# meyer-lab/cmtf-pls

Hardware: AMD Instinct MI355X
Metric: nipals_iters_per_sec (higher is better)
Workload: dtype f32

## Files before the change

cmtf_pls_amd/_lib.py:

```python
from __future__ import annotations

import ctypes
import os
from ctypes import c_char_p, c_double, c_int, c_int64, c_size_t, c_uint32, c_uint64, c_void_p

_HERE = os.path.dirname(os.path.abspath(__file__))
LIB_PATH = os.environ.get("CMTFPLS_LIB") or os.path.join(_HERE, "lib", "libcmtfpls.so")

_P = c_void_p

class XcovBlock(ctypes.Structure):
    _fields_ = [("S", _P), ("S2", _P), ("colcnt", _P), ("n_samples", c_double), ("order", c_int), ("A", c_int), ("B", c_int),
                ("n_squarings", c_int), ("Z", _P), ("wA", _P), ("wB", _P), ("info", _P)]


class KfoldState(ctypes.Structure):
    _fields_ = [("I", c_int), ("A", c_int), ("B", c_int), ("M", c_int), ("K", c_int), ("R", c_int)] + [
        (name, _P) for name in ("fold_of", "S", "mean", "Yk", "Gy", "WA", "WB", "Q", "Wa", "Wb", "T", "Gt", "coef", "Rm", "tm",
                                "Tout", "vec", "n_iter", "status", "part")]


class CvCoupledBlock(ctypes.Structure):
    _fields_ = [("X", _P), ("order", c_int), ("A", c_int), ("B", c_int)]


class LooCoupledBlock(ctypes.Structure):
    _fields_ = [("X", _P), ("colsum", _P), ("order", c_int), ("A", c_int), ("B", c_int)]


SIGNATURES = {
    "cmtfpls_xcov_iterate_blocks_f64": (c_int, [ctypes.POINTER(XcovBlock), c_int, c_int, _P, _P, _P, _P, _P, c_int, _P, c_size_t, _P]),
    "cmtfpls_abi_version": (c_int, []),
    "cmtfpls_last_error": (c_char_p, []),
    "cmtfpls_clear_error": (c_int, []),
    "cmtfpls_status_to_host": (c_int, [_P, _P, c_size_t, _P, _P]),
    "cmtfpls_colstats_workspace_bytes": (c_size_t, [c_int64, c_int64]),
    "cmtfpls_colstats_f32": (c_int, [_P, c_int64, c_int64, _P, _P, _P, c_size_t, _P]),
    "cmtfpls_colstats_f64": (c_int, [_P, c_int64, c_int64, _P, _P, _P, c_size_t, _P]),
    "cmtfpls_sweep_partials": (c_int, []),
    "cmtfpls_center_f32": (c_int, [_P, c_int64, c_int64, _P, _P, _P, _P]),
    "cmtfpls_center_f64": (c_int, [_P, c_int64, c_int64, _P, _P, _P, _P]),
    "cmtfpls_mode0_contract_workspace_bytes": (c_size_t, [c_int64, c_int64]),
# ... 144 lines not shown
                                                                       c_int, c_int]),
    "cmtfpls_loo_xcov_coupled_tensor_lds_bytes": (c_size_t, [ctypes.POINTER(LooCoupledBlock), c_int, ctypes.POINTER(c_int), c_int, c_int,
                                                            c_int]),
    "cmtfpls_loo_xcov_coupled_tensor_f64": (c_int, [ctypes.POINTER(LooCoupledBlock), c_int, ctypes.POINTER(c_int), _P, _P, c_int, c_int, c_int,
                                                    c_double, c_int, c_int, c_int, _P, _P, _P, c_size_t, _P]),
    "cmtfpls_cv_masked_fold_workspace_bytes": (c_size_t, [c_int, c_int, c_int, c_int, c_int]),
    "cmtfpls_cv_masked_f64": (c_int, [_P, _P, _P, c_int, _P, _P, _P, c_int, c_int, c_int, c_int, c_int, c_double, c_int, c_int,
                                      c_int, _P, _P, _P, _P, _P, c_size_t, _P]),
    "cmtfpls_cv_masked_model_workspace_bytes": (c_size_t, [c_int, c_int, c_int, c_int, c_int]),
    "cmtfpls_cv_masked_models_f64": (c_int, [_P, _P, _P, _P, c_int, c_int, c_int, c_int, c_int, c_int, c_double, c_int, c_int, c_int]
                                     + [_P] * 8 + [_P, c_size_t, _P]),
    "cmtfpls_cv_masked_tensor_fold_workspace_bytes": (c_size_t, [c_int] * 6),
    "cmtfpls_cv_masked_tensor_f64": (c_int, [_P, _P, _P, c_int, _P, _P, _P, c_int, c_int, c_int, c_int, c_int, c_int, c_double, c_int,
                                             c_int, c_int, _P, _P, _P, _P, _P, c_size_t, _P]),
    "cmtfpls_cv_masked_tensor_model_workspace_bytes": (c_size_t, [c_int] * 6),
    "cmtfpls_cv_masked_tensor_models_f64": (c_int, [_P, _P, _P, _P, c_int, c_int, c_int, c_int, c_int, c_int, c_int, c_double, c_int,
                                                    c_int, c_int] + [_P] * 9 + [_P, c_size_t, _P]),
    "cmtfpls_cv_masked_coupled_workspace_bytes": (c_size_t, [ctypes.POINTER(CvCoupledBlock), c_int, c_int, c_int, c_int]),
    "cmtfpls_cv_masked_coupled_lds_bytes": (c_size_t, [ctypes.POINTER(CvCoupledBlock), c_int, c_int, c_int, c_int]),
    "cmtfpls_cv_masked_coupled_f64": (c_int, [ctypes.POINTER(CvCoupledBlock), c_int, _P, _P, _P, c_int, c_int, c_int, c_int, c_double,
                                              c_int, c_int, c_int] + [_P] * 8 + [_P, c_size_t, _P]),
    "cmtfpls_fit_small_workspace_bytes": (c_size_t, [c_int, c_int, c_int, c_int]),
    "cmtfpls_fit_small_f64": (c_int, [_P, _P, c_int, c_int, c_int, c_int, c_int, c_double, c_int] + [_P] * 11 + [_P, c_size_t, _P]),
    "cmtfpls_add_noise_f32": (c_int, [_P, c_int64, c_double, c_uint64, c_uint64, c_double, _P]),
    "cmtfpls_add_noise_f64": (c_int, [_P, c_int64, c_double, c_uint64, c_uint64, c_double, _P]),
    "cmtfpls_ceiling_max_blocks": (c_int, []),
    "cmtfpls_ceiling_read": (c_int, [_P, c_size_t, c_int64, c_int, _P, c_int, _P]),
    "cmtfpls_ceiling_rmw": (c_int, [_P, c_size_t, c_int64, c_int, c_int, _P]),
    "cmtfpls_ceiling_copy": (c_int, [_P, _P, c_size_t, c_int64, c_int, c_int, _P]),
}

_lib = None


class CmtfplsError(RuntimeError):
    pass


def load():
    global _lib
    if _lib is not None:
        return _lib
    if not os.path.exists(LIB_PATH):
        raise CmtfplsError(
            f"{LIB_PATH} not found: build the HIP extension first (python -c 'import __graft_entry__ as g; g.build()'). "
            "cmtf_pls_amd has no CPU fallback."
# ... 15 lines not shown
```

cmtf_pls_amd/backend.py:

```python
from __future__ import annotations

import ctypes
from typing import Optional, Tuple

import torch

from . import _lib

_SUFFIX = {torch.float32: "f32", torch.float64: "f64"}


def _ptr(t: Optional[torch.Tensor]):
    return None if t is None else t.data_ptr()


def _int_pairs(pairs):
    flat = [int(v) for p in pairs for v in p]
    return (ctypes.c_int * len(flat))(*flat)


def _scratch(nbytes: int, device) -> torch.Tensor:
    return torch.empty(max(int(nbytes), 256), dtype=torch.uint8, device=device)


# ... 318 lines not shown
        return self._form(rc, "mttkrp", out)

    def score(self, X2, A, B, wA, wB, rowcnt, out) -> torch.Tensor:
        _lib.check(self._fn("score", X2)(_ptr(X2), X2.shape[0], A, B, _ptr(wA), _ptr(wB), _ptr(rowcnt), _ptr(out), self._stream()), "score")
        return out

    def score_s(self, S, A, B, wA, wB, out) -> torch.Tensor:
        assert S.dtype == torch.float64 and S.is_contiguous()
        _lib.check(self.lib.cmtfpls_score_s_f64(_ptr(S), S.shape[0], A, B, _ptr(wA), _ptr(wB), _ptr(out), self._stream()), "score_s")
        return out

    def score_contract(self, X2, A, B, wA, wB, shift, t, Z, sub_own=None, add_other=None, alpha: float = 1.0,
                       csum: Optional[torch.Tensor] = None) -> Optional[torch.Tensor]:
        I, P = X2.shape
        if not X2.is_contiguous() or P != A * B:
            return None
        for v in (sub_own, add_other):
            assert v is None or (v.is_contiguous() and v.numel() == I and v.dtype == torch.float64)
        nbytes = self.lib.cmtfpls_score_contract_workspace_bytes(I, P)
        ws = self._workspace("score_contract", max(nbytes, 256))
        rc = self._fn("score_contract", X2)(_ptr(X2), I, A, B, _ptr(wA), _ptr(wB), _ptr(shift), _ptr(sub_own), _ptr(add_other), float(alpha),
                                            _ptr(t), _ptr(Z), _ptr(csum), _ptr(ws), ws.numel(), self._stream())
        return self._form(rc, "score_contract", Z)

    def score_gram(self, X2, A, B, wA, wB, rowcnt, out, Y: torch.Tensor, qpart: torch.Tensor) -> Optional[torch.Tensor]:
        assert qpart.numel() >= self.n_partials * Y.shape[1] and qpart.is_contiguous()
        rc = self._fn("score_gram", X2)(_ptr(X2), X2.shape[0], A, B, _ptr(wA), _ptr(wB), _ptr(rowcnt), _ptr(out),
                                        _ptr(Y), Y.stride(0), Y.shape[1], _ptr(qpart), self._stream())
        return self._form(rc, "score_gram", out)

    def q_update(self, q: torch.Tensor, qpart: Optional[torch.Tensor] = None, normalize: bool = True,
                 G: Optional[torch.Tensor] = None, q_prev: Optional[torch.Tensor] = None,
                 du2: Optional[torch.Tensor] = None, nparts: Optional[int] = None) -> None:
        M = q.numel()
        nrows = (nparts or self.n_partials) if qpart is not None else 0
        assert qpart is None or (qpart.is_contiguous() and qpart.numel() >= nrows * M)
        _lib.check(self.lib.cmtfpls_q_update_f64(_ptr(qpart), nrows, M, _ptr(q), int(normalize),
                                                 _ptr(G), _ptr(q_prev), _ptr(du2), self._stream()), "q_update")

    def deflate(self, X2, A, B, t, wA, wB) -> torch.Tensor:
        part = self.empty(self.n_partials)
        _lib.check(self._fn("deflate", X2)(_ptr(X2), X2.shape[0], A, B, _ptr(t), _ptr(wA), _ptr(wB), _ptr(part), self._stream()), "deflate")
        return self._close_partials(part)

    def deflate_contract_yq(self, X2, A, B, t, wA, wB, Y: torch.Tensor, q: torch.Tensor, masked: bool,
                            out: torch.Tensor) -> Optional[torch.Tensor]:
# ... 543 lines not shown
```

cmtf_pls_amd/fitrun.py:

```python
from __future__ import annotations

import math
from typing import Dict, List, Optional

import numpy as np
import torch

from .fitrun_xcov import XcovMixin
from .state import BlockState, FitState, split_trailing, validate_limits


class FitRun(XcovMixin):

    def __init__(self, eng: NipalsEngine, Xs: List[torch.Tensor], Y: torch.Tensor, n_components: int, coupled: bool,
                 algorithm: str = "direct", owned: Optional[List[bool]] = None, allow_raw: bool = True):
        be, comm = eng.be, eng.comm
        Xs = list(Xs)
        owned = [True] * len(Xs) if owned is None else list(owned)
        if algorithm not in ("direct", "xcov"):
            raise ValueError("algorithm must be 'direct' or 'xcov'")
        self.algorithm_requested = self.algorithm = algorithm
        self.notes: List[str] = []
        validate_limits([tuple(X.shape) for X in Xs], n_components)
        self.eng, self.Xs, self.Y, self.R, self.coupled = eng, Xs, Y, n_components, coupled
# ... 105 lines not shown
            self.S, self.S2, self.S12 = [], [], []
            for blk in self.blocks:
                if blk.has_miss and self._s_pair:
                    both = be.empty(2 * M, blk.A * blk.B)
                    self.S12.append(both)
                    self.S.append(both[:M])
                    self.S2.append(both[M:])
                else:
                    self.S12.append(None)
                    pre = self._s_prebuilt.get(len(self.S))
                    self.S.append(pre if pre is not None else be.empty(M, blk.A * blk.B))
                    self.S2.append(be.empty(M, blk.A * blk.B) if blk.has_miss else None)
            self.rowscale = [(float(blk.A * blk.B) / blk.rowcnt) if blk.has_miss else None for blk in self.blocks]
            any_miss = any(blk.has_miss for blk in self.blocks)
            self.Yw = be.empty(I, 2 * M if self._s_pair else M) if any_miss else None
            self.Gy = be.empty(M, M)
            self.Tq = be.empty(nb, M)
            self.qx = [be.zeros(M), be.zeros(M)]
            self.qc = self.qx[0]
            self.qn = self.Tq[0] if (nb == 1 and not coupled) else be.empty(M)
            self._s_carry = (not any(blk.has_miss for blk in self.blocks)
                             and all(hasattr(be, f) for f in ("s_downdate", "deflate_contract_yq")))
            self._s_ready = False
            self._nowrite = False
            if self.raw:
                self.zM = be.zeros(M)
                self.zA = [be.zeros(blk.A) for blk in self.blocks]
                self.zB = [be.zeros(blk.B) for blk in self.blocks]
            if self._s_carry:
                self.yhat = be.empty(I, 1)
                self.one = be.empty(1)
                self.one.fill_(1.0)
                self.vs = [be.empty(blk.A * blk.B) for blk in self.blocks]
                self._nowrite = eng.opt.xcov_nowrite and hasattr(be, "kr_axpy") and R <= 64
                if self._nowrite:
                    self.dot_log = be.zeros(R, 1 + len(self.blocks))
                    self.Gw = be.empty(R * R)
                    self._G_last = None
                    self._one_read = R > 1 and eng.opt.xcov_one_read and hasattr(be, "score_contract")
                    if self._one_read:
                        self._fused_b = max(range(len(self.blocks)), key=lambda b: self.blocks[b].A * self.blocks[b].B)
                        P0 = self.blocks[self._fused_b].A * self.blocks[self._fused_b].B
                        self.ps = be.empty(P0)
                        self.Rm = be.zeros(P0, R)
                        self.corr = be.empty(I)
                        self.csum = be.empty(1)
            assert self._nowrite or not self.raw, "an uncentred X needs the form of the loop that never writes it"

    def _blocks_from_one_read(self, Xs: List[torch.Tensor]) -> Optional[List[BlockState]]:
        be, comm = self.eng.be, self.eng.comm
        blocks, n = [], float(self.n_total)
        for b, X in enumerate(Xs):
            I = X.shape[0]
            X2 = X.view(I, -1)
            P = X2.shape[1]
            out = be.xcov_stats(X2, self.Y, out=be.empty(self.M, P))
            if out is None:
                return None
            S, stats = out
            comm.allreduce(stats)
            colsum, colsq = stats[:P], stats[P:]
            ssq = (colsq - colsum * colsum / n).sum().reshape(1)
            if not bool(torch.isfinite(ssq).all().item()):
                return None
            A, B = split_trailing(X.shape)
            blocks.append(BlockState(shape=tuple(X.shape), A=A, B=B, mean=colsum / n, has_miss=False, colcnt=None, rowcnt=None,
                                     ssq0=float("nan"), dtype=X.dtype))
            self._s_prebuilt[b] = S
            self._ssq0_dev[b] = ssq
        return blocks
# ... 17 lines not shown
            if self.S12[b] is not None:
                self.Yw[:, :self.M].copy_(self.Y)
                torch.mul(self.Y, self.rowscale[b][:, None], out=self.Yw[:, self.M:])
                be.xcov(self.X2[b], self.Yw, True, out=self.S12[b], mixed=self.mixed)
                comm.allreduce(self.S12[b])
                continue
            if b in self._s_prebuilt:
                del self._s_prebuilt[b]
            elif self.raw and self._ssq_with_s and b not in self._ssq0_dev:
                _, ssq = be.xcov_ssq(self.X2[b], self.Y, blk.mean, out=self.S[b])
                self._ssq0_dev[b] = comm.allreduce(ssq)
            else:
                be.xcov(self.X2[b], self.Y, blk.has_miss, out=self.S[b], mixed=self.mixed)
            comm.allreduce(self.S[b])
            if self.raw:
                ysum, _ = be.colstats(self.Y)
                comm.allreduce(ysum)
                be.s_downdate(self.S[b], blk.A, blk.B, self.zM, self.zA[b], self.zB[b], ysum, blk.mean)
            if blk.has_miss:
                torch.mul(self.Y, self.rowscale[b][:, None], out=self.Yw)
                be.xcov(self.X2[b], self.Yw, True, out=self.S2[b], mixed=self.mixed)
                comm.allreduce(self.S2[b])
        self._s_ready = False
        be.gram_tn(self.Y, self.Y, out=self.Gy)
        comm.allreduce(self.Gy)
        self._parity = 0
        self.qc = self.qx[0]
        self.qc.zero_()
        self.qc[0] = 1.0

    def inner_loop(self, a: int, max_iter: int, tol: float, verbose: int = 0) -> None:
        if max_iter > 0 and self._pipeline_ok():
            self._pipelined = True
            self._inner_loop_xcov_pipelined(a, max_iter, tol, verbose)
            return
        for it in range(max_iter):
            du = self.iterate(it)
            if du is not None and du < tol:
                if verbose:
                    print("Comp {}: converged after {} iterations".format(a, it))
                break

    def _update_budgets(self, host) -> bool:
        retry = False
        for b in range(len(self.blocks)):
            conv, used = host[1 + 2 * b] > 0.5, int(host[2 + 2 * b])
            if used < 0:
                self._chain_gave_up()
                retry = True
                continue
# ... 349 lines not shown
    def _store_loadings(self, a: int) -> None:
        for b, blk in enumerate(self.blocks):
            if len(blk.shape) == 2:
                blk.loadings[0][:, a].copy_(self.wB[b])
            elif len(blk.shape) == 3:
                blk.loadings[0][:, a].copy_(self.wA[b])
                blk.loadings[1][:, a].copy_(self.wB[b])
            else:
                for m, d in enumerate(blk.shape[1:]):
                    blk.loadings[m][:, a].copy_(self.fac[b][m, :d])

    def result(self) -> FitState:
        if getattr(self, "_state", None) is not None:
            return self._state
        nb = len(self.blocks)
        nowrite = self.algorithm == "xcov" and getattr(self, "_nowrite", False)
        for b, ssq in getattr(self, "_ssq0_dev", {}).items():
            self.blocks[b].ssq0 = float(ssq.item())
        self.eng.comm.allreduce(self.ssq_log)
        parts = [self.coef_dev.reshape(-1), self.ssq_log.reshape(-1)]
        if nowrite:
            self.eng.comm.allreduce(self.dot_log)
            parts.append(self.dot_log.reshape(-1))
        host = torch.cat(parts).cpu().numpy()
        R = self.R
        self.coef[...] = host[: R * R].reshape(R, R)
        ssq = host[R * R: R * R + R * (nb + 1)].reshape(R, nb + 1).copy()
        if nowrite:
            dots = host[R * R + R * (nb + 1):].reshape(R, 1 + nb)
            for b, blk in enumerate(self.blocks):
                run = blk.ssq0
                for a in range(len(self.n_iter)):
                    run = run - 2.0 * dots[a, 1 + b] + dots[a, 0]
                    ssq[a, b] = run
        for a in range(len(self.n_iter)):
            for b, blk in enumerate(self.blocks):
                blk.r2x[a] = 1.0 - ssq[a, b] / blk.ssq0
            self.r2y[a] = 1.0 - ssq[a, nb] / self.ssqy0
        self._state = FitState(coupled=self.coupled, n_components=self.R, blocks=self.blocks, T=self.T, U=self.U, Q=self.Q,
                               coef=self.coef, r2y=self.r2y, y_mean=self.y_mean, n_iter=self.n_iter,
                               n_samples_total=self.n_total, report=self.build_report())
        return self._state

    def build_report(self) -> Dict[str, object]:
        eng, comm, nb = self.eng, self.eng.comm, len(self.blocks)
        rep: Dict[str, object] = {
            "form": "regular", "algorithm_requested": self.algorithm_requested, "algorithm": self.algorithm,
            "shapes": [tuple(b.shape) for b in self.blocks], "storage": [str(b.dtype).replace("torch.", "") for b in self.blocks],
            "missing": [bool(b.has_miss) for b in self.blocks], "responses": self.M,
            "sharded": bool(comm.sharded), "world": int(comm.world),
            "graphs": bool(self.use_graphs and self._graphs), "graph_error": self._graph_error,
            "collectives_in_graph": self._collectives_captured is True,
# ... 9 lines not shown
            rep["x_copy"] = "centred private copy"
        else:
            nowrite = bool(getattr(self, "_nowrite", False))
            one_read = nowrite and bool(getattr(self, "_one_read", False))
            any_miss = any(b.has_miss for b in self.blocks)
            rep["x_copy"] = "none: the caller's uncentred tensor is read in place" if self.raw else "centred private copy"
            rep["raw"] = bool(self.raw)
            rep["x_written"] = not nowrite
            rep["s_carried"] = bool(self._s_carry)
            rep["s_build"] = ("per component (missing values)" if any_miss else "first component only") + \
                             (f", {(self.M + 63) // 64} response tiles of <= 64" if self.M > 64 else "") + \
                             (", [Y, Y * rowscale] in one pass" if any(x is not None for x in self.S12) else "")
            rep["one_read"] = one_read
            rep["stats_with_s"] = bool(getattr(self, "_stats_with_s", False))
            if nowrite:
                rep["x_passes_per_component"] = ("1 read (largest block); 2 reads (other blocks)" if one_read and nb > 1 else
                                                 "1 read" if one_read else "2 reads")
            elif any_miss and nb == 1 and getattr(self, "_deflate_build_ok", True) and self.S12[0] is not None and eng.opt.xcov_deflate_build:
                rep["x_passes_per_component"] = "1 read + 1 read + write (deflation inside the rebuild of S)"
            elif any_miss:
                rep["x_passes_per_component"] = "1 read + write (score + deflation) + S rebuild reads"
            else:
                rep["x_passes_per_component"] = "1 read + 1 read + write"
            rep["pipelined"] = bool(getattr(self, "_pipelined", False))
            if rep["pipelined"]:
                rep["pipeline"] = dict(self.pipeline_stats)
            if not rep["pipelined"] and eng.opt.xcov_pipeline:
                why = ("graph replay requested" if self.use_graphs else "more than 64 responses" if self.M > 64 else
                       "a block of order > 3 or a backend without the single-call iteration")
                self.notes.append("inner loop on S not pipelined: " + why)
            if self.algorithm_requested == "xcov" and not self.raw and eng.opt.xcov_raw and not any_miss and not any("uncentred" in n for n in self.notes):
                self.notes.append("uncentred xcov form declined: " + ("more than 64 components" if self.R > 64 else
                                                                      "f32 matrix precision or a backend without its kernels"))
            if nowrite and eng.opt.xcov_one_read and self.R > 1 and not one_read:
                self.notes.append("one read per component declined: the row does not fit the registers of 1..16 workgroups "
                                  "(rows of 2048..131072 f32 -- 262144 when the last mode divides 4096 -- / 1024..131072 f64 elements, "
                                  "last mode a multiple of 4 / 2)")
        rep["rank1_one_launch_chain"] = bool(getattr(eng.be, "rank1_chain_side", 0)) and any(
            len(blk.shape) == 3 and min(blk.A, blk.B) <= int(getattr(eng.be, "rank1_chain_side", 0)) for blk in self.blocks)
        rep["declined"] = list(self.notes)
        return rep
```

cmtf_pls_amd/fitrun_xcov.py:

```python
from __future__ import annotations

import math
from typing import Optional

import torch


class XcovMixin:
    def _iterate_xcov(self, it: int) -> Optional[float]:
        be = self.eng.be
        self._executed += 1

        blk0 = self.blocks[0]
        composite = (len(self.blocks) == 1 and len(blk0.shape) == 3 and not blk0.has_miss and self.M <= 64
                     and self.qn.data_ptr() == self.Tq.data_ptr() and hasattr(be, "xcov_iterate"))

        par = self._parity
        q_cur, q_new = self.qx[par], self.qx[par ^ 1]

        def seg(first: bool):
            if composite:
                be.xcov_iterate(self.S[0], blk0.A, blk0.B, q_cur, self.Zs[0], self.wA[0], self.wB[0], self.status[1:3],
                                self.sq_budget[0], q_new, self.Gy, self.status[0:1], first)
                return
# ... 169 lines not shown
        ssqs = []
        if k < self.R:
            be.rowdot(Ta, b_dev, self.yhat.view(-1), None)
        ssqy = be.y_deflate(self.Y, self.T, k, b_dev, self.q)
        if k < self.R:
            carried = True
            for b, blk in enumerate(self.blocks):
                s_b = be.deflate_contract_yq(self.X2[b], blk.A, blk.B, self.t, self.wA[b], self.wB[b], self.yhat, self.one,
                                             False, out=self.vs[b])
                if s_b is None:
                    s_b = be.deflate(self.X2[b], blk.A, blk.B, self.t, self.wA[b], self.wB[b])
                    carried = False
                ssqs.append(s_b)
            if carried:
                for b, blk in enumerate(self.blocks):
                    comm.allreduce(self.vs[b])
                    be.s_downdate(self.S[b], blk.A, blk.B, ya_g, self.wA[b], self.wB[b], self.q, self.vs[b])
            self._s_ready = carried
        else:
            for b, blk in enumerate(self.blocks):
                ssqs.append(be.deflate(self.X2[b], blk.A, blk.B, self.t, self.wA[b], self.wB[b]))
        self._log_ssq(a, ssqs, ssqy)

    def _finish_xcov_nowrite(self, a: int) -> None:
        be, comm = self.eng.be, self.eng.comm
        self.q = self.qc
        I, R, k = self.I, self.R, a + 1
        nb = len(self.blocks)
        self._store_loadings(a)
        fused_b = self._fused_b if (getattr(self, "_one_read", False) and k < R) else -1
        one_read = False
        for b in [x for x in range(nb) if x != fused_b] + ([fused_b] if fused_b >= 0 else []):
            blk = self.blocks[b]
            mw = None
            if self.raw:
                mw = be.score_s(blk.mean.view(1, -1), blk.A, blk.B, self.wA[b], self.wB[b], be.empty(1))
            g = None
            if a > 0 and hasattr(be, "kr_gram_row"):
                for m, L in enumerate(blk.loadings):
                    be.kr_gram_row(L, a, self.Gw, first=(m == 0))
                g = self.Gw[:a]
            elif a > 0:
                for m, L in enumerate(blk.loadings):
                    be.kr_gram(L, self.Gw, first=(m == 0))
                g = self.Gw.view(R, R)[a, :a]
            if b == fused_b:
                corr = others = None
                if a > 0:
                    be.rowdot(self.T[:, :a], g, self.corr, None)
                    corr = self.corr
                if nb == 2:
# ... 54 lines not shown
```

cmtf_pls_amd/options.py:

```python
from __future__ import annotations

from dataclasses import dataclass, replace
from typing import Optional


@dataclass(frozen=True)
class EngineOptions:
    small_fit: bool = True
    small_fit_elements: int = 1 << 15
    xcov_nowrite: bool = True
    xcov_raw: bool = True
    xcov_raw_max_offset: float = 1e4
    project_raw_max_offset: float = 1e4
    xcov_one_read: bool = True
    xcov_pair_build: bool = True
    xcov_ssq_with_s: bool = True
    xcov_stats_with_s: bool = True
    xcov_deflate_build: bool = True
    xcov_pipeline: bool = True
    capture_collectives: bool = False
    project_split_rows: bool = True
    masked_folds: bool = False
    masked_folds_coupled: bool = False
    coupled_permutations: bool = False
    tensor_folds: bool = False
    tensor_folds_coupled: bool = False
    masked_tensor_folds: bool = False
    tensor_resamples_coupled: bool = False

    def but(self, **changes) -> "EngineOptions":
        return replace(self, **changes)


_DEFAULT_OPTIONS = EngineOptions()


def default_options() -> EngineOptions:
    return _DEFAULT_OPTIONS


def set_default_options(options: Optional[EngineOptions]) -> EngineOptions:
    global _DEFAULT_OPTIONS
# ... 3 lines not shown
```

include/cmtfpls.h:

```cpp
#ifndef CMTFPLS_H
#define CMTFPLS_H

#include <stddef.h>
#include <stdint.h>

#ifdef __cplusplus
extern "C" {
#endif

#define CMTFPLS_OK 0
#define CMTFPLS_EINVAL 1
#define CMTFPLS_EWORKSPACE 2
#define CMTFPLS_EHIP 3
#define CMTFPLS_EUNSUPPORTED 4

int cmtfpls_abi_version(void);
const char* cmtfpls_last_error(void);
int cmtfpls_clear_error(void);
int cmtfpls_status_to_host(const void* src, void* dst_host, size_t bytes, void* event, void* stream);

size_t cmtfpls_colstats_workspace_bytes(int64_t I, int64_t P);
int cmtfpls_colstats_f32(const float* X, int64_t I, int64_t P, double* colsum, double* colcnt,
                         void* ws, size_t ws_bytes, void* stream);
int cmtfpls_colstats_f64(const double* X, int64_t I, int64_t P, double* colsum, double* colcnt,
// ... 332 lines not shown
int cmtfpls_kfold_inner_grouped_f64(const cmtfpls_kfold_state* st, const int* model_fold, int groups, int a, double tol, int max_iter,
                                    void* ws, size_t ws_bytes, void* stream);
int cmtfpls_kfold_epilogue_grouped_f64(const cmtfpls_kfold_state* st, const int* model_fold, int groups, int stage, int a, const double* in,
                                       void* stream);
int cmtfpls_kfold_inner_coupled_grouped_f64(const cmtfpls_kfold_state* blocks, int nb, const int* model_fold, int groups, int a, double tol,
                                            int max_iter, void* ws, size_t ws_bytes, void* stream);

int cmtfpls_kfold_epilogue_splits_f64(const cmtfpls_kfold_state* st, int splits, int stage, int a, const double* in, void* stream);

size_t cmtfpls_kfold_weighted_xcov_workspace_bytes(int64_t I, int64_t P, int n, int M);
int cmtfpls_kfold_weighted_xcov_f32(const float* X, int64_t I, int A, int B, const double* Y, int n, int M, double* S, double* mean,
                                    double* stats, void* ws, size_t ws_bytes, void* stream);
int cmtfpls_kfold_weighted_xcov_f64(const double* X, int64_t I, int A, int B, const double* Y, int n, int M, double* S, double* mean,
                                    double* stats, void* ws, size_t ws_bytes, void* stream);
int cmtfpls_kfold_epilogue_weighted_f64(const cmtfpls_kfold_state* st, int stage, int a, const double* in, void* stream);
size_t cmtfpls_press_rows_workspace_bytes(int n, int64_t I, int R, int M);
int cmtfpls_press_rows_f64(const double* T, const double* coef, const double* Q, const double* nu, const double* Y, const int* eval,
                           int n, int64_t I, int R, int M, double* press, double* pred, void* ws, size_t ws_bytes, void* stream);
size_t cmtfpls_fit_small_workspace_bytes(int I, int A, int B, int M);
int cmtfpls_fit_small_f64(const double* X, const double* Y, int I, int A, int B, int M, int R, double tol, int max_iter,
                          double* T, double* U, double* WA, double* WB, double* Q, double* coef, double* ssq, double* x_mean,
                          double* y_mean, int* n_iter, int* flag, void* ws, size_t ws_bytes, void* stream);

int cmtfpls_add_noise_f32(float* X, int64_t n, double sigma, uint64_t seed, uint64_t offset, double nan_fraction,
                          void* stream);
int cmtfpls_add_noise_f64(double* X, int64_t n, double sigma, uint64_t seed, uint64_t offset, double nan_fraction,
                          void* stream);

int cmtfpls_ceiling_max_blocks(void);
int cmtfpls_ceiling_read(const void* buf, size_t bytes, int64_t row_bytes, int map, float* sink, int blocks, void* stream);
int cmtfpls_ceiling_rmw(void* buf, size_t bytes, int64_t row_bytes, int map, int blocks, void* stream);
int cmtfpls_ceiling_copy(const void* src, void* dst, size_t bytes, int64_t row_bytes, int map, int blocks, void* stream);

#ifdef __cplusplus
}
#endif
#endif
```

Before: 766.9.

## Fuse the component-boundary work of the no-write xcov fit into dedicated kernels

Adds a HIP module that folds the per-component boundary of the no-write cross-covariance NIPALS fit into a few kernels: gram-row correction, score/response stats, a small normal-equation solve, Y deflation with Gram accumulation, and the S downdate. The one-read score-contract X pass runs between the staged kernels. It also carries the Y Gram into the next component so it is not recomputed. The aim is to cut many small launches and host round trips between components. It adds a parallel code path with size limits (M, R ≤ 64, single order-3 block) and falls back when the shape is not supported.

```diff
diff --git a/cmtf_pls_amd/_lib.py b/cmtf_pls_amd/_lib.py
--- a/cmtf_pls_amd/_lib.py
+++ b/cmtf_pls_amd/_lib.py
@@ -18,6 +18,13 @@
     _fields_ = [("I", c_int), ("A", c_int), ("B", c_int), ("M", c_int), ("K", c_int), ("R", c_int)] + [
         (name, _P) for name in ("fold_of", "S", "mean", "Yk", "Gy", "WA", "WB", "Q", "Wa", "Wb", "T", "Gt", "coef", "Rm", "tm",
                                 "Tout", "vec", "n_iter", "status", "part")]
+
+
+class XcovFitState(ctypes.Structure):
+    _fields_ = [("X", _P)] + [(name, c_int) for name in ("I", "A", "B", "M", "R", "raw")] + [
+        (name, _P) for name in ("Y", "T", "U", "Q", "LA", "LB", "wA", "wB", "q", "q0", "mean", "S", "Rm", "coef", "Gt", "Gy", "dot_log",
+                                "ssq_log", "t", "ps", "corr", "csum", "vec", "part")] + [
+        ("part_bytes", c_size_t), ("pass_ws", _P), ("pass_ws_bytes", c_size_t), ("status", _P)]
 
 
 class CvCoupledBlock(ctypes.Structure):
@@ -208,6 +215,10 @@
                                               c_int, c_int, c_int] + [_P] * 8 + [_P, c_size_t, _P]),
     "cmtfpls_fit_small_workspace_bytes": (c_size_t, [c_int, c_int, c_int, c_int]),
     "cmtfpls_fit_small_f64": (c_int, [_P, _P, c_int, c_int, c_int, c_int, c_int, c_double, c_int] + [_P] * 11 + [_P, c_size_t, _P]),
+    "cmtfpls_xcov_boundary_row_tiles": (c_int, [c_int64]),
+    "cmtfpls_xcov_boundary_workspace_bytes": (c_size_t, [c_int64, c_int, c_int]),
+    "cmtfpls_xcov_boundary_f32": (c_int, [ctypes.POINTER(XcovFitState), c_int, c_int, _P]),
+    "cmtfpls_xcov_boundary_f64": (c_int, [ctypes.POINTER(XcovFitState), c_int, c_int, _P]),
     "cmtfpls_add_noise_f32": (c_int, [_P, c_int64, c_double, c_uint64, c_uint64, c_double, _P]),
     "cmtfpls_add_noise_f64": (c_int, [_P, c_int64, c_double, c_uint64, c_uint64, c_double, _P]),
     "cmtfpls_ceiling_max_blocks": (c_int, []),
diff --git a/cmtf_pls_amd/backend.py b/cmtf_pls_amd/backend.py
--- a/cmtf_pls_amd/backend.py
+++ b/cmtf_pls_amd/backend.py
@@ -364,6 +364,61 @@
         rc = self._fn("score_contract", X2)(_ptr(X2), I, A, B, _ptr(wA), _ptr(wB), _ptr(shift), _ptr(sub_own), _ptr(add_other), float(alpha),
                                             _ptr(t), _ptr(Z), _ptr(csum), _ptr(ws), ws.numel(), self._stream())
         return self._form(rc, "score_contract", Z)
+
+    def xcov_boundary_state(self, X2: torch.Tensor, A: int, B: int, raw: bool, **buf) -> "_lib.XcovFitState":
+        assert X2.is_contiguous() and X2.dtype in _SUFFIX and X2.shape[1] == A * B
+        I, M = buf["Y"].shape
+        R = buf["T"].shape[1]
+        buf = dict(buf)
+        for name, make in (("Gt", lambda: self.zeros(R, R)), ("vec", lambda: self.zeros(3 * R + M + 2)), ("status", lambda: self.zeros(1)),
+                           ("part", lambda: self.zeros(max(1, self.lib.cmtfpls_xcov_boundary_workspace_bytes(I, M, R) // 8)))):
+            if buf.get(name) is None:
+                buf[name] = make()
+        pass_ws = None
+        if R > 1:
+            pass_ws = self._workspace("score_contract", max(self.lib.cmtfpls_score_contract_workspace_bytes(I, A * B), 256))
+        st = _lib.XcovFitState()
+        st.X, st.I, st.A, st.B, st.M, st.R, st.raw = _ptr(X2), I, A, B, M, R, int(bool(raw))
+        for name in ("Y", "T", "U", "Q", "LA", "LB", "wA", "wB", "q", "q0", "mean", "S", "Rm", "coef", "Gt", "Gy", "dot_log", "ssq_log", "t",
+                     "ps", "corr", "csum", "vec", "part", "status"):
+            v = buf.get(name)
+            assert v is None or (v.is_contiguous() and v.dtype == torch.float64 and v.device == self.device), name
+            setattr(st, name, _ptr(v))
+        st.part_bytes = buf["part"].numel() * 8
+        st.pass_ws, st.pass_ws_bytes = _ptr(pass_ws), (pass_ws.numel() if pass_ws is not None else 0)
+        st.tensors = dict(buf, X=X2, pass_ws=pass_ws)
+        st.fn = self._fn("xcov_boundary", X2)
+        return st
+
+    def xcov_boundary(self, state, a: int, q: Optional[torch.Tensor] = None, stages: int = 63, pass_here: bool = False) -> Optional[bool]:
+        if q is not None:
+            assert q.is_contiguous() and q.dtype == torch.float64 and q.numel() == state.M
+            state.q = _ptr(q)
+            state.tensors["q"] = q
+        if not (pass_here and stages == 63):
+            return self._form(state.fn(ctypes.byref(state), int(a), int(stages), self._stream()), "xcov_boundary")
+        t, R, M = state.tensors, state.R, state.M
+        X2, last = t["X"], a + 1 == R
+        if not last:
+            if getattr(state, "pass_ok", None) is None:
+                rc = self._fn("score_contract", X2)(_ptr(X2), state.I, state.A, state.B, _ptr(t["wA"]), _ptr(t["wB"]), None, None, None, 1.0,
+                                                    _ptr(t["t"]), _ptr(t["ps"]), None, None, 0, self._stream())
+                state.pass_ok = rc == 2
+            if not state.pass_ok:
+                return None
+        _lib.check(state.fn(ctypes.byref(state), int(a), 1, self._stream()), "xcov_boundary (stage A)")
+        if last:
+            self.score(X2, state.A, state.B, t["wA"], t["wB"], None, t["t"])
+        else:
+            raw = bool(state.raw)
+            mw = t["vec"][3 * R + M + 1:] if raw else None
+            if self.score_contract(X2, state.A, state.B, t["wA"], t["wB"], mw, t["t"], t["ps"], sub_own=t["corr"] if a > 0 else None,
+                                   csum=t["csum"] if raw else None) is None:
+                return None
+        return self._form(state.fn(ctypes.byref(state), int(a), 4 | 8 | 16 | 32, self._stream()), "xcov_boundary")
+
+    def xcov_boundary_row_tiles(self, I: int) -> int:
+        return int(self.lib.cmtfpls_xcov_boundary_row_tiles(I))
 
     def score_gram(self, X2, A, B, wA, wB, rowcnt, out, Y: torch.Tensor, qpart: torch.Tensor) -> Optional[torch.Tensor]:
         assert qpart.numel() >= self.n_partials * Y.shape[1] and qpart.is_contiguous()
diff --git a/cmtf_pls_amd/csrc/xcov_boundary.hip b/cmtf_pls_amd/csrc/xcov_boundary.hip
--- /dev/null
+++ b/cmtf_pls_amd/csrc/xcov_boundary.hip
@@ -0,0 +1,350 @@
+#include "common.hpp"
+#include "fold_regress.hpp"
+
+namespace cmtfpls {
+
+constexpr int kXbThreads = 256, kXbPrepThreads = 1024, kXbSolveThreads = 1024, kXbMaxTiles = 256, kXbMaxM = 64, kXbMaxR = 64, kXbChunk = 32, kXbRespPerBlock = 4;
+constexpr int kXbPartStride = 2 * kXbMaxR + 1 + kXbMaxM;
+enum XbStage : int { kXbStageA = 1, kXbStagePass = 2, kXbStageB1 = 4, kXbStageB2 = 8, kXbStageB3 = 16, kXbStageC = 32 };
+
+__host__ __device__ inline int xb_tiles(int64_t I) {
+  int64_t nt = (I + kXbThreads - 1) / kXbThreads;
+  return (int)(nt > kXbMaxTiles ? kXbMaxTiles : (nt < 1 ? 1 : nt));
+}
+
+__device__ __forceinline__ void xb_tile_rows(int I, int NT, int tile, int* lo, int* hi) {
+  const int len = (I + NT - 1) / NT;
+  *lo = min(I, tile * len);
+  *hi = min(I, (tile + 1) * len);
+}
+
+__host__ __device__ inline int xb_vec_len(int R, int M) { return 3 * R + M + 2; }
+
+__device__ __forceinline__ void xb_gram_row(const cmtfpls_xcov_fit_state& st, int a, double* g) {
+  const int lane = threadIdx.x & 63, wv = threadIdx.x >> 6, R = st.R;
+  for (int j = wv; j < a; j += kXbPrepThreads / 64) {
+    double sa = 0.0, sb = 0.0;
+    for (int i = lane; i < st.A; i += 64) sa = fma(st.LA[(int64_t)i * R + j], st.wA[i], sa);
+    for (int i = lane; i < st.B; i += 64) sb = fma(st.LB[(int64_t)i * R + j], st.wB[i], sb);
+    sa = wave_sum(sa);
+    sb = wave_sum(sb);
+    if (lane == 0) g[j] = sa * sb;
+  }
+  __syncthreads();
+}
+
+__global__ __launch_bounds__(kXbPrepThreads) void xb_prepare_kernel(cmtfpls_xcov_fit_state st, int a) {
+  __shared__ double g[kXbMaxR];
+  __shared__ double slot[16];
+  const int tid = threadIdx.x, R = st.R, M = st.M;
+  xb_gram_row(st, a, g);
+  if (blockIdx.x + 1 == gridDim.x) {
+    double* vec = st.vec;
+    for (int i = tid; i < st.A; i += kXbPrepThreads) st.LA[(int64_t)i * R + a] = st.wA[i];
+    for (int i = tid; i < st.B; i += kXbPrepThreads) st.LB[(int64_t)i * R + a] = st.wB[i];
+    for (int j = tid; j < a; j += kXbPrepThreads) vec[2 * R + M + 1 + j] = g[j];
+    double s = 0.0;
+    if (st.raw) {
+      const int64_t P = (int64_t)st.A * st.B;
+      KronWalk kw(tid, kXbPrepThreads, st.B);
+      for (int64_t c = tid; c < P; c += kXbPrepThreads) {
+        s = fma(st.mean[c], st.wA[kw.j] * st.wB[kw.k], s);
+        kw.next();
+      }
+      s = block_sum(s, slot);
+    }
+    if (tid == 0) vec[3 * R + M + 1] = s;
+    return;
+  }
+  int lo, hi;
+  xb_tile_rows(st.I, (int)gridDim.x - 1, (int)blockIdx.x, &lo, &hi);
+  for (int i = lo + tid; i < hi; i += kXbPrepThreads) {
+    double s = 0.0;
+    for (int j = 0; j < a; ++j) s = fma(st.T[(int64_t)i * R + j], g[j], s);
+    st.corr[i] = s;
+  }
+}
+
+template <bool FIXUP>
+__global__ __launch_bounds__(kXbThreads) void xb_rows_kernel(cmtfpls_xcov_fit_state st, int a) {
+  constexpr int NW = kXbThreads / 64;
+  __shared__ double acc[NW][kXbPartStride];
+  __shared__ double q[kXbMaxM], g[kXbMaxR];
+  const int tid = threadIdx.x, lane = tid & 63, wv = tid >> 6, tile = blockIdx.x;
+  const int I = st.I, M = st.M, R = st.R, kk = a + 1, NT = (int)gridDim.x, nv = 2 * kk + 1 + M;
+  const double mw = FIXUP ? st.vec[3 * R + M + 1] : 0.0;
+  for (int m = tid; m < M; m += kXbThreads) q[m] = st.q[m];
+  if (FIXUP)
+    for (int j = tid; j < a; j += kXbThreads) g[j] = st.vec[2 * R + M + 1 + j];
+  for (int v = tid; v < NW * kXbPartStride; v += kXbThreads) (&acc[0][0])[v] = 0.0;
+  __syncthreads();
+  int lo, hi;
+  xb_tile_rows(I, NT, tile, &lo, &hi);
+  for (int i0 = lo; i0 < hi; i0 += kXbThreads) {
+    const int i = i0 + tid;
+    const bool ok = i < hi;
+    double t = 0.0, u = 0.0;
+    if (ok) {
+      t = st.t[i];
+      if (FIXUP) {
+        t -= mw;
+        for (int j = 0; j < a; ++j) t = fma(-st.T[(int64_t)i * R + j], g[j], t);
+        st.t[i] = t;
+      }
+      for (int m = 0; m < M; ++m) u = fma(st.Y[(int64_t)i * M + m], q[m], u);
+      st.T[(int64_t)i * R + a] = t;
+      st.U[(int64_t)i * R + a] = u;
+    }
+    for (int p = 0; p < kk; ++p) {
+      const double tp = ok ? (p == a ? t : st.T[(int64_t)i * R + p]) : 0.0;
+      const double s1 = wave_sum(tp * t), s2 = wave_sum(tp * u);
+      if (lane == 0) { acc[wv][p] += s1; acc[wv][kk + p] += s2; }
+    }
+    const double s3 = wave_sum(t);
+    if (lane == 0) acc[wv][2 * kk] += s3;
+    for (int m = 0; m < M; ++m) {
+      const double s4 = wave_sum(ok ? st.Y[(int64_t)i * M + m] * t : 0.0);
+      if (lane == 0) acc[wv][2 * kk + 1 + m] += s4;
+    }
+  }
+  __syncthreads();
+  for (int v = tid; v < nv; v += kXbThreads) {
+    double s = 0.0;
+    for (int w = 0; w < NW; ++w) s += acc[w][v];
+    st.part[(int64_t)tile * kXbPartStride + v] = s;
+  }
+}
+
+__device__ __forceinline__ double xb_tiles_sum(const double* __restrict__ p, int NT, int64_t stride, int lane) {
+  double s = 0.0;
+  for (int t = lane; t < NT; t += 64) s += p[(int64_t)t * stride];
+  return wave_sum(s);
+}
+
+__global__ __launch_bounds__(kXbSolveThreads) void xb_solve_kernel(cmtfpls_xcov_fit_state st, int a, int NT) {
+  __shared__ double tot[kXbPartStride];
+  __shared__ double Gn[kXbMaxR * kXbMaxR];
+  __shared__ double bb[kXbMaxR], dd[kXbMaxR];
+  const int tid = threadIdx.x, lane = tid & 63, wv = tid >> 6;
+  const int M = st.M, R = st.R, kk = a + 1, nv = 2 * kk + 1 + M;
+  double* Gt = st.Gt;
+  double* vec = st.vec;
+  for (int v = wv; v < nv; v += kXbSolveThreads / 64) {
+    const double s = xb_tiles_sum(st.part + v, NT, kXbPartStride, lane);
+    if (lane == 0) tot[v] = s;
+  }
+  for (int m = tid; m < M; m += kXbSolveThreads) st.Q[(int64_t)m * R + a] = st.q[m];
+  __syncthreads();
+  auto G = [&](int i, int j) { return i == a ? tot[j] : (j == a ? tot[i] : Gt[i * R + j]); };
+  for (int o = tid; o < kk * kk; o += kXbSolveThreads) Gn[o] = G(o / kk, o % kk);
+  for (int m = tid; m < M; m += kXbSolveThreads) vec[2 * R + m] = tot[2 * kk + 1 + m];
+  if (tid == 0) {
+    vec[2 * R + M] = tot[2 * kk];
+    st.dot_log[2 * a] = tot[a];
+    st.dot_log[2 * a + 1] = tot[a];
+  }
+  __syncthreads();
+  if (tid == 0) {
+    fold_normal_solve(Gn, tot + kk, kk, dd, bb);
+    if (!isfinite(bb[a]) || !isfinite(tot[2 * kk])) st.status[0] = 1.0;
+  }
+  __syncthreads();
+  for (int r = tid; r < kk; r += kXbSolveThreads) { st.coef[(int64_t)r * R + a] = bb[r]; vec[r] = bb[r]; }
+  for (int r = wv; r < kk; r += kXbSolveThreads / 64) {
+    const double v = wave_sum(lane < kk ? G(r, lane) * bb[lane] : 0.0);
+    if (lane == 0) vec[R + r] = v;
+  }
+  for (int p = tid; p < kk; p += kXbSolveThreads) { Gt[a * R + p] = tot[p]; Gt[p * R + a] = tot[p]; }
+}
+
+__global__ __launch_bounds__(kXbThreads) void xb_ydefl_kernel(cmtfpls_xcov_fit_state st, int a) {
+  constexpr int EPT = kXbMaxM * kXbMaxM / kXbThreads;
+  __shared__ double Ys[kXbChunk][kXbMaxM + 1];
+  __shared__ double yh[kXbChunk];
+  __shared__ double q[kXbMaxM], b[kXbMaxR];
+  const int tid = threadIdx.x, tile = blockIdx.x;
+  const int I = st.I, M = st.M, R = st.R, kk = a + 1, NT = (int)gridDim.x;
+  for (int m = tid; m < M; m += kXbThreads) q[m] = st.Q[(int64_t)m * R + a];
+  for (int j = tid; j < kk; j += kXbThreads) b[j] = st.vec[j];
+  __syncthreads();
+  double* gpart = st.part + (int64_t)NT * kXbPartStride;
+  double accg[EPT];
+#pragma unroll
+  for (int e = 0; e < EPT; ++e) accg[e] = 0.0;
+  int lo, hi;
+  xb_tile_rows(I, NT, tile, &lo, &hi);
+  for (int i0 = lo; i0 < hi; i0 += kXbChunk) {
+    if (tid < kXbChunk) {
+      const int i = i0 + tid;
+      double s = 0.0;
+      if (i < hi)
+        for (int j = 0; j < kk; ++j) s = fma(st.T[(int64_t)i * R + j], b[j], s);
+      yh[tid] = s;
+    }
+    __syncthreads();
+    for (int idx = tid; idx < kXbChunk * M; idx += kXbThreads) {
+      const int r = idx / M, m = idx % M, i = i0 + r;
+      double y = 0.0;
+      if (i < hi) {
+        y = fma(-yh[r], q[m], st.Y[(int64_t)i * M + m]);
+        st.Y[(int64_t)i * M + m] = y;
+      }
+      Ys[r][m] = y;
+    }
+    __syncthreads();
+#pragma unroll
+    for (int e = 0; e < EPT; ++e) {
+      const int o = tid + e * kXbThreads;
+      if (o < M * M) {
+        const int m1 = o / M, m2 = o % M;
+        double s = accg[e];
+        for (int r = 0; r < kXbChunk; ++r) s = fma(Ys[r][m1], Ys[r][m2], s);
+        accg[e] = s;
+      }
+    }
+    __syncthreads();
+  }
+#pragma unroll
+  for (int e = 0; e < EPT; ++e) {
+    const int o = tid + e * kXbThreads;
+    if (o < M * M) gpart[(int64_t)tile * M * M + o] = accg[e];
+  }
+}
+
+__global__ __launch_bounds__(kXbThreads) void xb_close_kernel(cmtfpls_xcov_fit_state st, int a, int NT, int ncb, int ndd, int ngy) {
+  __shared__ double diag[kXbMaxM];
+  const int tid = threadIdx.x, lane = tid & 63, wv = tid >> 6, M = st.M, R = st.R;
+  const double* gpart = st.part + (int64_t)NT * kXbPartStride;
+  const int blk = (int)blockIdx.x;
+  if (blk >= ndd + ngy) {
+    for (int m = wv; m < M; m += kXbThreads / 64) {
+      const double s = xb_tiles_sum(gpart + (int64_t)m * M + m, NT, (int64_t)M * M, lane);
+      if (lane == 0) diag[m] = s;
+    }
+    for (int m = tid; m < M; m += kXbThreads) st.q0[m] = (m == 0) ? 1.0 : 0.0;
+    __syncthreads();
+    if (tid == 0) {
+      double s = 0.0;
+      for (int m = 0; m < M; ++m) s += diag[m];
+      st.ssq_log[2 * a + 1] = s;
+    }
+    return;
+  }
+  if (blk >= ndd) {
+    const int o = (blk - ndd) * (kXbThreads / 64) + wv;
+    if (o < M * M) {
+      const double s = xb_tiles_sum(gpart + o, NT, (int64_t)M * M, lane);
+      if (lane == 0) st.Gy[o] = s;
+    }
+    return;
+  }
+  const int cb = blk % ncb, mg = blk / ncb;
+  const int64_t P = (int64_t)st.A * st.B, c = (int64_t)cb * kXbThreads + tid;
+  if (c >= P) return;
+  const double* vec = st.vec;
+  const int ia = (int)(c / st.B), ib = (int)(c % st.B);
+  double r = st.ps[c];
+  if (st.raw) r -= st.csum[0] * st.mean[c];
+  if (mg == 0) st.Rm[c * R + a] = r;
+  double v = 0.0;
+  for (int j = 0; j < a; ++j) v = fma(vec[j], st.Rm[c * R + j], v);
+  v = fma(vec[a], r, v);
+  for (int j = 0; j <= a; ++j) v = fma(-vec[R + j], st.LA[(int64_t)ia * R + j] * st.LB[(int64_t)ib * R + j], v);
+  const double w = st.LA[(int64_t)ia * R + a] * st.LB[(int64_t)ib * R + a];
+  const int m1 = min(M, (mg + 1) * kXbRespPerBlock);
+  for (int m = mg * kXbRespPerBlock; m < m1; ++m) st.S[(int64_t)m * P + c] -= fma(w, vec[2 * R + m], v * st.Q[(int64_t)m * R + a]);
+}
+
+static int xb_pass(const float* X, int64_t I, int A, int B, const double* wA, const double* wB, const double* shift, const double* sub,
+                   double* t, double* Z, double* csum, void* ws, size_t wsb, void* s) {
+  return cmtfpls_score_contract_f32(X, I, A, B, wA, wB, shift, sub, nullptr, 1.0, t, Z, csum, ws, wsb, s);
+}
+static int xb_pass(const double* X, int64_t I, int A, int B, const double* wA, const double* wB, const double* shift, const double* sub,
+                   double* t, double* Z, double* csum, void* ws, size_t wsb, void* s) {
+  return cmtfpls_score_contract_f64(X, I, A, B, wA, wB, shift, sub, nullptr, 1.0, t, Z, csum, ws, wsb, s);
+}
+static int xb_score(const float* X, int64_t I, int A, int B, const double* wA, const double* wB, double* t, void* s) {
+  return cmtfpls_score_f32(X, I, A, B, wA, wB, nullptr, t, s);
+}
+static int xb_score(const double* X, int64_t I, int A, int B, const double* wA, const double* wB, double* t, void* s) {
+  return cmtfpls_score_f64(X, I, A, B, wA, wB, nullptr, t, s);
+}
+
+template <typename T>
+static int run_xcov_boundary(const cmtfpls_xcov_fit_state* sp, int a, int stages, void* stream) {
+  if (!sp) { set_error("xcov_boundary: bad argument"); return CMTFPLS_EINVAL; }
+  const cmtfpls_xcov_fit_state& s = *sp;
+  if (s.I <= 0 || s.A <= 0 || s.B <= 0 || s.M <= 0 || s.R <= 0 || a < 0 || a >= s.R || stages <= 0 || stages > 63) {
+    set_error("xcov_boundary: bad argument");
+    return CMTFPLS_EINVAL;
+  }
+  const int64_t P = (int64_t)s.A * s.B;
+  if (s.M > kXbMaxM || s.R > kXbMaxR || s.I > ((int64_t)1 << 30) || P >= ((int64_t)1 << 31)) {
+    set_error("xcov_boundary: shape outside the fused form (M <= 64, R <= 64, I <= 2^30); use the launch-by-launch boundary");
+    return CMTFPLS_EUNSUPPORTED;
+  }
+  const bool last = a + 1 == s.R;
+  if (!s.X || !s.Y || !s.T || !s.U || !s.Q || !s.LA || !s.LB || !s.wA || !s.wB || !s.q || !s.q0 || !s.coef || !s.Gt || !s.Gy ||
+      !s.dot_log || !s.ssq_log || !s.t || !s.vec || !s.part || !s.status || (s.raw && !s.mean) ||
+      (s.R > 1 && (!s.S || !s.Rm || !s.ps || !s.corr || (s.raw && !s.csum)))) {
+    set_error("xcov_boundary: a buffer of the state is missing");
+    return CMTFPLS_EINVAL;
+  }
+  const int NT = xb_tiles(s.I);
+  if (s.part_bytes < cmtfpls_xcov_boundary_workspace_bytes(s.I, s.M, s.R)) {
+    set_error("xcov_boundary: tile workspace too small");
+    return CMTFPLS_EWORKSPACE;
+  }
+  const T* X = static_cast<const T*>(s.X);
+  double* mwp = s.vec + 3 * s.R + s.M + 1;
+  if ((stages & kXbStagePass) && !last) {
+    const int rc = xb_pass(X, s.I, s.A, s.B, s.wA, s.wB, nullptr, nullptr, s.t, s.ps, nullptr, nullptr, 0, stream);
+    if (rc != CMTFPLS_EWORKSPACE) return rc ? rc : CMTFPLS_EINVAL;
+    if (!s.pass_ws || s.pass_ws_bytes < cmtfpls_score_contract_workspace_bytes(s.I, P)) {
+      set_error("xcov_boundary: workspace of the pass too small");
+      return CMTFPLS_EWORKSPACE;
+    }
+  }
+  hipStream_t st = (hipStream_t)stream;
+  if (stages & kXbStageA) {
+    const bool corr = a > 0 && !last;
+    hipLaunchKernelGGL(xb_prepare_kernel, dim3(corr ? NT + 1 : 1), dim3(kXbPrepThreads), 0, st, s, a);
+  }
+  if (stages & kXbStagePass) {
+    int rc;
+    if (last) rc = xb_score(X, s.I, s.A, s.B, s.wA, s.wB, s.t, stream);
+    else rc = xb_pass(X, s.I, s.A, s.B, s.wA, s.wB, s.raw ? mwp : nullptr, a > 0 ? s.corr : nullptr, s.t, s.ps, s.raw ? s.csum : nullptr,
+                      s.pass_ws, s.pass_ws_bytes, stream);
+    if (rc) return rc;
+  }
+  if (stages & kXbStageB1) {
+    if (last) hipLaunchKernelGGL(xb_rows_kernel<true>, dim3(NT), dim3(kXbThreads), 0, st, s, a);
+    else hipLaunchKernelGGL(xb_rows_kernel<false>, dim3(NT), dim3(kXbThreads), 0, st, s, a);
+  }
+  if (stages & kXbStageB2) hipLaunchKernelGGL(xb_solve_kernel, dim3(1), dim3(kXbSolveThreads), 0, st, s, a, NT);
+  if (stages & kXbStageB3) hipLaunchKernelGGL(xb_ydefl_kernel, dim3(NT), dim3(kXbThreads), 0, st, s, a);
+  if (stages & kXbStageC) {
+    const int ncb = (int)((P + kXbThreads - 1) / kXbThreads), ngr = (s.M + kXbRespPerBlock - 1) / kXbRespPerBlock;
+    const int ndd = last ? 0 : ncb * ngr, ngy = (s.M * s.M + kXbThreads / 64 - 1) / (kXbThreads / 64);
+    hipLaunchKernelGGL(xb_close_kernel, dim3((unsigned)(ndd + ngy + 1)), dim3(kXbThreads), 0, st, s, a, NT, ncb, ndd, ngy);
+  }
+  return check_launch("xcov_boundary");
+}
+
+}
+
+using namespace cmtfpls;
+
+extern "C" {
+int cmtfpls_xcov_boundary_row_tiles(int64_t I) { return I > 0 ? xb_tiles(I) : 0; }
+size_t cmtfpls_xcov_boundary_workspace_bytes(int64_t I, int M, int R) {
+  if (I <= 0 || M <= 0 || R <= 0) return 0;
+  return (size_t)xb_tiles(I) * ((size_t)kXbPartStride + (size_t)M * M) * sizeof(double);
+}
+int cmtfpls_xcov_boundary_f32(const cmtfpls_xcov_fit_state* state, int a, int stages, void* stream) {
+  return run_xcov_boundary<float>(state, a, stages, stream);
+}
+int cmtfpls_xcov_boundary_f64(const cmtfpls_xcov_fit_state* state, int a, int stages, void* stream) {
+  return run_xcov_boundary<double>(state, a, stages, stream);
+}
+}
diff --git a/cmtf_pls_amd/fitrun.py b/cmtf_pls_amd/fitrun.py
--- a/cmtf_pls_amd/fitrun.py
+++ b/cmtf_pls_amd/fitrun.py
@@ -151,6 +151,10 @@
             self._s_carry = (not any(blk.has_miss for blk in self.blocks)
                              and all(hasattr(be, f) for f in ("s_downdate", "deflate_contract_yq")))
             self._s_ready = False
+            self._gy_ready = False
+            self._boundary = None
+            self._boundary_runs = 0
+            self._boundary_why = None
             self._nowrite = False
             if self.raw:
                 self.zM = be.zeros(M)
@@ -174,7 +178,43 @@
                         self.Rm = be.zeros(P0, R)
                         self.corr = be.empty(I)
                         self.csum = be.empty(1)
+                    self._boundary_setup(coupled)
             assert self._nowrite or not self.raw, "an uncentred X needs the form of the loop that never writes it"
+
+    def _boundary_setup(self, coupled: bool) -> None:
+        be, comm, eng = self.eng.be, self.eng.comm, self.eng
+        if not hasattr(be, "xcov_boundary"):
+            return
+        blk = self.blocks[0]
+        why = None
+        if not eng.opt.xcov_fused_boundary:
+            self._boundary_why = "xcov_fused_boundary = False"
+            return
+        if len(self.blocks) != 1 or coupled:
+            why = "coupled blocks"
+        elif len(blk.shape) != 3:
+            why = "a block of order %d" % len(blk.shape)
+        elif blk.has_miss:
+            why = "missing values"
+        elif comm.sharded:
+            why = "a sharded fit"
+        elif self.M > 64 or self.R > 64:
+            why = "more than 64 responses or components"
+        elif self.X2[0].dtype not in (torch.float32, torch.float64) or not self.X2[0].is_contiguous():
+            why = "X is not contiguous f32 / f64"
+        elif self.R > 1 and not self._one_read:
+            why = "the one-read pass is switched off (xcov_one_read = False)"
+        if why is not None:
+            self._boundary_why = why
+            self.notes.append("fused component boundary declined: " + why)
+            return
+        one = self.R > 1
+        self._boundary = be.xcov_boundary_state(
+            self.X2[0], blk.A, blk.B, self.raw, Y=self.Y, T=self.T, U=self.U, Q=self.Q, LA=blk.loadings[0], LB=blk.loadings[1],
+            wA=self.wA[0], wB=self.wB[0], q=self.qx[0], q0=self.qx[0], mean=blk.mean if self.raw else None, S=self.S[0] if one else None,
+            Rm=self.Rm if one else None, coef=self.coef_dev, Gy=self.Gy, dot_log=self.dot_log, ssq_log=self.ssq_log, t=self.t,
+            ps=self.ps if one else None, corr=self.corr if one else None, csum=self.csum if (one and self.raw) else None)
+        self._boundary_status = self._boundary.tensors["status"]
 
     def _blocks_from_one_read(self, Xs: List[torch.Tensor]) -> Optional[List[BlockState]]:
         be, comm = self.eng.be, self.eng.comm
@@ -238,10 +278,13 @@
                 be.xcov(self.X2[b], self.Yw, True, out=self.S2[b], mixed=self.mixed)
                 comm.allreduce(self.S2[b])
         self._s_ready = False
+        self._parity = 0
+        self.qc = self.qx[0]
+        if self._gy_ready:
+            self._gy_ready = False
+            return
         be.gram_tn(self.Y, self.Y, out=self.Gy)
         comm.allreduce(self.Gy)
-        self._parity = 0
-        self.qc = self.qx[0]
         self.qc.zero_()
         self.qc[0] = 1.0
 
@@ -637,12 +680,17 @@
         if nowrite:
             self.eng.comm.allreduce(self.dot_log)
             parts.append(self.dot_log.reshape(-1))
+        fused_runs = getattr(self, "_boundary_runs", 0)
+        if fused_runs:
+            parts.append(self._boundary_status)
         host = torch.cat(parts).cpu().numpy()
+        if fused_runs:
+            self._boundary_nonfinite = bool(host[-1] != 0.0)
         R = self.R
         self.coef[...] = host[: R * R].reshape(R, R)
         ssq = host[R * R: R * R + R * (nb + 1)].reshape(R, nb + 1).copy()
         if nowrite:
-            dots = host[R * R + R * (nb + 1):].reshape(R, 1 + nb)
+            dots = host[R * R + R * (nb + 1): R * R + 2 * R * (nb + 1)].reshape(R, 1 + nb)
             for b, blk in enumerate(self.blocks):
                 run = blk.ssq0
                 for a in range(len(self.n_iter)):
@@ -698,6 +746,12 @@
                 rep["x_passes_per_component"] = "1 read + write (score + deflation) + S rebuild reads"
             else:
                 rep["x_passes_per_component"] = "1 read + 1 read + write"
+            if hasattr(eng.be, "xcov_boundary"):
+                rep["boundary"] = {"fused": self._boundary_runs > 0, "components": self._boundary_runs,
+                                   "form": ("fused: stage A, the X pass, stages B1, B2, B3 and C (csrc/xcov_boundary.hip)"
+                                            if self._boundary_runs else "launch by launch"),
+                                   "declined": self._boundary_why,
+                                   "nonfinite": bool(getattr(self, "_boundary_nonfinite", False))}
             rep["pipelined"] = bool(getattr(self, "_pipelined", False))
             if rep["pipelined"]:
                 rep["pipeline"] = dict(self.pipeline_stats)
diff --git a/cmtf_pls_amd/fitrun_xcov.py b/cmtf_pls_amd/fitrun_xcov.py
--- a/cmtf_pls_amd/fitrun_xcov.py
+++ b/cmtf_pls_amd/fitrun_xcov.py
@@ -215,11 +215,23 @@
                 ssqs.append(be.deflate(self.X2[b], blk.A, blk.B, self.t, self.wA[b], self.wB[b]))
         self._log_ssq(a, ssqs, ssqy)
 
+    def _finish_xcov_boundary(self, a: int) -> bool:
+        if self.eng.be.xcov_boundary(self._boundary, a, q=self.qc, pass_here=True) is None:
+            self._boundary = None
+            self._boundary_why = "the one-read pass does not take the shape"
+            self.notes.append("fused component boundary declined: " + self._boundary_why)
+            return False
+        self._boundary_runs += 1
+        self._s_ready = self._gy_ready = a + 1 < self.R
+        return True
+
     def _finish_xcov_nowrite(self, a: int) -> None:
         be, comm = self.eng.be, self.eng.comm
         self.q = self.qc
         I, R, k = self.I, self.R, a + 1
         nb = len(self.blocks)
+        if self._boundary is not None and self._finish_xcov_boundary(a):
+            return
         self._store_loadings(a)
         fused_b = self._fused_b if (getattr(self, "_one_read", False) and k < R) else -1
         one_read = False
diff --git a/cmtf_pls_amd/options.py b/cmtf_pls_amd/options.py
--- a/cmtf_pls_amd/options.py
+++ b/cmtf_pls_amd/options.py
@@ -18,6 +18,7 @@
     xcov_stats_with_s: bool = True
     xcov_deflate_build: bool = True
     xcov_pipeline: bool = True
+    xcov_fused_boundary: bool = True
     capture_collectives: bool = False
     project_split_rows: bool = True
     masked_folds: bool = False
diff --git a/include/cmtfpls.h b/include/cmtfpls.h
--- a/include/cmtfpls.h
+++ b/include/cmtfpls.h
@@ -378,6 +378,44 @@
                           double* T, double* U, double* WA, double* WB, double* Q, double* coef, double* ssq, double* x_mean,
                           double* y_mean, int* n_iter, int* flag, void* ws, size_t ws_bytes, void* stream);
 
+typedef struct cmtfpls_xcov_fit_state {
+  const void* X;
+  int I, A, B, M, R;
+  int raw;
+  double* Y;
+  double* T;
+  double* U;
+  double* Q;
+  double* LA;
+  double* LB;
+  const double* wA;
+  const double* wB;
+  const double* q;
+  double* q0;
+  const double* mean;
+  double* S;
+  double* Rm;
+  double* coef;
+  double* Gt;
+  double* Gy;
+  double* dot_log;
+  double* ssq_log;
+  double* t;
+  double* ps;
+  double* corr;
+  double* csum;
+  double* vec;
+  double* part;
+  size_t part_bytes;
+  void* pass_ws;
+  size_t pass_ws_bytes;
+  double* status;
+} cmtfpls_xcov_fit_state;
+int cmtfpls_xcov_boundary_row_tiles(int64_t I);
+size_t cmtfpls_xcov_boundary_workspace_bytes(int64_t I, int M, int R);
+int cmtfpls_xcov_boundary_f32(const cmtfpls_xcov_fit_state* state, int a, int stages, void* stream);
+int cmtfpls_xcov_boundary_f64(const cmtfpls_xcov_fit_state* state, int a, int stages, void* stream);
+
 int cmtfpls_add_noise_f32(float* X, int64_t n, double sigma, uint64_t seed, uint64_t offset, double nan_fraction,
                           void* stream);
 int cmtfpls_add_noise_f64(double* X, int64_t n, double sigma, uint64_t seed, uint64_t offset, double nan_fraction,
```

Result: no change. 767.7, median of 2 (+0.1%).
